# arclab-hku/ESVIO

Measured on AMD Instinct MI355X. Metric: Mevents/s through time-surface+detect+track @640x480, higher is better.
Workload: dtype f64 timestamps / u8 images / f32 LK sums in the reference build's order

## Files before the change

### esvio_amd/csrc/fe_kernels.hip

```cpp
#include "fe_kernels.h"
#include "fe_mc.h"

#include <algorithm>
#include <cstdio>
#include <cstdlib>
#include <cstring>
#include <tuple>
#include <type_traits>

namespace esvio {

namespace {
template <typename... P, typename... A>
void launch_k(void (*kernel)(P...), dim3 grid, dim3 block, unsigned shmem, hipStream_t s, A... args) {
  static_assert(sizeof...(P) == sizeof...(A), "argument count");
  hipLaunchKernelGGL(kernel, grid, block, shmem, s, args...);
}
}

__device__ __forceinline__ int lane_id() { return threadIdx.x & 63; }

__device__ __forceinline__ double ev_time(uint32_t sec, uint32_t nsec) {
  return __dadd_rn((double)sec, __dmul_rn(1e-9, (double)nsec));
}
// ... 1739 lines not shown
  float scale, corr;
};
__device__ __forceinline__ RedLane red_lane(int lane) {
  RedLane r;
  r.take_b = (lane & 2) != 0;
  const bool hi = (lane & 1) != 0;
  r.off = hi ? 12u : 0u;
  r.wid = hi ? 20u : 12u;
  r.scale = hi ? 0x1p-8f : 0x1p-20f;
  r.corr = hi ? -(float)(1 << 22) * 0x1p-8f : 0.f;
  return r;
}
template <int CTRL>
__device__ __forceinline__ float quad_bcast(float v) {
  return __int_as_float(__builtin_amdgcn_update_dpp(0, __float_as_int(v), CTRL, 0xf, 0xf, true));
}
constexpr int kRedSeed = 1 << 28;
__device__ __forceinline__ void wave_sum2_exact(int a, int b, const RedLane& rl, float& fa, float& fb) {
  a = xor_add_dpp(a, 0xB1);
  b = xor_add_dpp(b, 0xB1);
  a = xor_add_dpp(a, 0x4E);
  b = xor_add_dpp(b, 0x4E);
  a = xor_add_dpp(a, 0x141);
  b = xor_add_dpp(b, 0x141);
  const uint32_t v = (uint32_t)(rl.take_b ? b : a);
  int x = (int)__builtin_amdgcn_ubfe(v, rl.off, rl.wid);
  x = xor_add_dpp(x, 0x128);
  x = xor16_add(x);
  x = xor32_add(x);
  const float t = __fmaf_rn((float)x, rl.scale, rl.corr);
  const float u = t + quad_bcast<0xB1>(t);
  fa = quad_bcast<0x00>(u);
  fb = quad_bcast<0xAA>(u);
}

typedef short ss2 __attribute__((ext_vector_type(2)));
typedef unsigned short us2 __attribute__((ext_vector_type(2)));
__device__ __forceinline__ uint32_t pack16(int lo, int hi) {
  return __builtin_amdgcn_perm((uint32_t)hi, (uint32_t)lo, 0x05040100u);
}
__device__ __forceinline__ int sdot2(uint32_t a, uint32_t b, int c) {
  return __builtin_amdgcn_sdot2(__builtin_bit_cast(ss2, a), __builtin_bit_cast(ss2, b), c, false);
}

__device__ __forceinline__ bool wave_any(bool c) { return __builtin_amdgcn_ballot_w64(c) != 0; }
typedef unsigned long long lanemask_t;
__device__ __forceinline__ lanemask_t bal(bool c) { return __builtin_amdgcn_ballot_w64(c); }

struct LkCall {
  PyrDesc P;
  PyrDesc N;
  int max_level;
  int max_count;
  double eps2;
  int flags;
};

struct LkRegionLane {
  int ry[(kLkRegDw + 63) / 64], rb[(kLkRegDw + 63) / 64];
};
__device__ __forceinline__ LkRegionLane lk_region_lane(int lane) {
  LkRegionLane r;
#pragma unroll
  for (int k = 0; k < (kLkRegDw + 63) / 64; k++) {
    const int d = min(k * 64 + lane, kLkRegDw - 1);
    r.ry[k] = d / (kLkRegW / 4);
    r.rb[k] = 4 * (d - r.ry[k] * (kLkRegW / 4));
  }
  return r;
}
__device__ __forceinline__ void lk_region_load(const uint8_t* J, int stride, int rows, int wx, int wy,
                                               int lane, const LkRegionLane& rl, int& rx0, int& ry0,
                                               uint32_t (&reg)[(kLkRegDw + 63) / 64]) {
  rx0 = (wx - kLkMargin) & ~3;
  ry0 = wy - kLkMargin;
  const int sx = __builtin_amdgcn_readfirstlane(rx0), sy = __builtin_amdgcn_readfirstlane(ry0);
  if (sx >= -kPad && sx + kLkRegW <= stride - kPad && sy >= -kPad && sy + kLkRegH <= rows + kPad) {
    const uint8_t* base = J + (ptrdiff_t)sy * stride + sx;
#pragma unroll
    for (int k = 0; k < (kLkRegDw + 63) / 64; k++) {
      uint32_t off;
      asm("v_mad_u32_u24 %0, %1, %2, %3" : "=v"(off) : "v"(rl.ry[k]), "s"(stride), "v"(rl.rb[k]));
      reg[k] = *(const uint32_t*)(base + off);
    }
    return;
  }
#pragma unroll
  for (int k = 0; k < (kLkRegDw + 63) / 64; k++) {
    int gy = ry0 + rl.ry[k], gx = rx0 + rl.rb[k];
    gy = min(max(gy, -kPad), rows + kPad - 1);
    gx = min(max(gx, -kPad), stride - kPad - 4);
    reg[k] = *(const uint32_t*)(J + (ptrdiff_t)gy * stride + gx);
  }
}
__device__ __forceinline__ void lk_region_store(uint32_t* regJ, int lane,
                                                const uint32_t (&reg)[(kLkRegDw + 63) / 64]) {
  __builtin_amdgcn_fence(__ATOMIC_SEQ_CST, "wavefront");
#pragma unroll
  for (int k = 0; k < (kLkRegDw + 63) / 64; k++) {
    regJ[k * 64 + lane] = reg[k];
  }
  __builtin_amdgcn_fence(__ATOMIC_SEQ_CST, "wavefront");
}

__device__ __forceinline__ float lk_chain_walk(const float* T) {
  float acc = 0.f;
  float c[5], nx[5];
#pragma unroll
  for (int q = 0; q < 5; q++) c[q] = T[q];
#pragma unroll
  for (int y = 0; y < kLkWin; y++) {
    const int yn = y + 1 < kLkWin ? y + 1 : y;
#pragma unroll
    for (int q = 0; q < 5; q++) nx[q] = T[yn * 5 + q];
#pragma unroll
    for (int q = 0; q < 5; q++) acc = __fadd_rn(acc, c[q]);
#pragma unroll
    for (int q = 0; q < 5; q++) c[q] = nx[q];
  }
  return acc;
}

constexpr int kLkChainsA = 15;
constexpr int kLkChainWordsA = kLkWin * 5;
constexpr int kLkTypeWordsA = 5 * kLkChainWordsA;
constexpr int kLkTermLevelA = kLkChainsA * kLkChainWordsA;
constexpr int kLkTermWordsA = kMaxLevels * kLkTermLevelA;
static_assert(kMaxLevels * 16 <= 64, "one DPP row of walkers per level");

typedef __attribute__((address_space(3))) float lds_f32;
__device__ __forceinline__ int lk_term_word_A(int row, int x) {
  const int chain = x < 16 ? (x & 3) : x < kLkWin ? 4 : (x & 3);
  const int slot = x < 16 ? (x >> 2) : x < kLkWin ? x - 16 : 4;
  return (chain * kLkWin + row) * 5 + slot;
}
template <int NP>
__device__ __forceinline__ void lk_float_terms_A(const uint32_t (&ta)[NP], int L, const int* pIx, const int* pIy) {
#pragma unroll
  for (int k = 0; k < NP; k++) {
    lds_f32* d = (lds_f32*)(uintptr_t)ta[k] + L * kLkTermLevelA;
    const float fx = (float)pIx[k], fy = (float)pIy[k];
    d[0] = __fmul_rn(fx, fx);
    d[kLkTypeWordsA] = __fmul_rn(fx, fy);
    d[2 * kLkTypeWordsA] = __fmul_rn(fy, fy);
  }
}
__device__ __forceinline__ float lk_float_walk_A(const float* TA, int lane) {
  __builtin_amdgcn_fence(__ATOMIC_SEQ_CST, "wavefront", "local");
  const int c = (lane & 15) < kLkChainsA ? (lane & 15) : 0;
  return lk_chain_walk(TA + ((lane >> 4) * kLkChainsA + c) * kLkChainWordsA);
}
template <int CTRL>
__device__ __forceinline__ float dpp_row_f32(float v) {
  return __int_as_float(__builtin_amdgcn_update_dpp(0, __float_as_int(v), CTRL, 0xf, 0xf, true));
}
__device__ __forceinline__ float lk_float_sums_A(float acc, float& a11, float& a12, float& a22) {
  const float kScale = 1.f / (float)(1 << 20);
  const float s1 = __fadd_rn(acc, dpp_row_f32<0x102>(acc));
  const float s2 = __fadd_rn(s1, dpp_row_f32<0x101>(s1));
  const float s3 = __fadd_rn(dpp_row_f32<0x104>(acc), s2);
  const float out = __fmul_rn(s3, kScale);
  a11 = out;
  a12 = dpp_row_f32<0x105>(out);
  a22 = dpp_row_f32<0x10A>(out);
  return out;
}

constexpr int kF32SegStore = 12;
constexpr int kF32VecSegs = 4, kF32VecTerms = 11;
constexpr int kF32TailSegs = 12, kF32TailTerms = 9;
constexpr int kF32VecWords = kF32VecSegs * kF32SegStore;
constexpr int kF32CompStride = 4 * kF32VecWords;
constexpr int kF32TailBase = 8 * kF32VecWords;
constexpr int kF32ZeroSeg = kF32TailBase + kF32TailSegs * kF32SegStore;
constexpr int kF32Dump = kF32TailBase + kF32CompStride + kF32TailSegs * kF32SegStore;
constexpr int kF32TermWords = kF32Dump + kF32CompStride + 64;
static_assert(kF32ZeroSeg + kF32SegStore <= kF32TailBase + kF32CompStride, "zero segment inside tail b1's padding");
constexpr unsigned long long kF32Walkers = 0x0FFFFFFFFFFF0FFFull;

struct LkLaneF32 {
  uint32_t wb[5];
  uint32_t rb;
  uint32_t ta[8];
  bool run2;
};
__device__ __forceinline__ LkLaneF32 lk_lane_f32(int lane_in, uint32_t ta_base ) {
  const int lane = lane_in < 63 ? lane_in : 62;
  LkLaneF32 r;
  const int row = lane / 3;
  const int run = lane - row * 3;
  r.run2 = run == 2;
#pragma unroll
  for (int k = 0; k < 8; k++) r.ta[k] = ta_base + 4u * (uint32_t)lk_term_word_A(row, run * 8 + k);
#pragma unroll
  for (int j = 0; j < 5; j++) {
    int w = kF32Dump + lane;
    if (run < 2 && j < 4) {
      const int idx = 2 * row + run;
      w = j * kF32VecWords + (idx / kF32VecTerms) * kF32SegStore + idx % kF32VecTerms;
    } else if (run == 2) {
      const int idx = 5 * row + j;
      w = kF32TailBase + (idx / kF32TailTerms) * kF32SegStore + idx % kF32TailTerms;
    }
    r.wb[j] = (uint32_t)w * 4u;
  }
  const int wrow = lane_in >> 4, l16 = lane_in & 15;
  int rw = kF32ZeroSeg;
  if (wrow == 0 || wrow == 3) {
    if (l16 < kF32TailSegs) rw = kF32TailBase + (wrow == 3 ? kF32CompStride : 0) + l16 * kF32SegStore;
  } else {
    rw = ((wrow - 1) * 4 + (l16 & 3)) * kF32VecWords + (l16 >> 2) * kF32SegStore;
  }
  r.rb = (uint32_t)rw * 4u;
  return r;
}
template <int CTRL, int ROWS, int BANKS>
__device__ __forceinline__ int dpp_add_masked(int v) {
  return v + __builtin_amdgcn_update_dpp(0, v, CTRL, ROWS, BANKS, false);
}

typedef __attribute__((address_space(3))) int lds_int;
typedef int i32x4 __attribute__((ext_vector_type(4)));
typedef __attribute__((address_space(3))) i32x4 lds_int4;

__device__ __forceinline__ void lk_float_sums_b(const int (&vx)[5], const int (&vy)[5], uint32_t tb, const LkLaneF32& ln,
                                                float& b1, float& b2) {
  __builtin_amdgcn_fence(__ATOMIC_SEQ_CST, "wavefront", "local");
#pragma unroll
  for (int j = 0; j < 5; j++) {
    lds_int* d = (lds_int*)(uintptr_t)(tb + ln.wb[j]);
    d[0] = vx[j];
    d[kF32CompStride] = vy[j];
  }
  __builtin_amdgcn_fence(__ATOMIC_SEQ_CST, "wavefront", "local");
  int t[kF32SegStore];
  {
    const lds_int4* src = (const lds_int4*)(uintptr_t)(tb + ln.rb);
#pragma unroll
    for (int q = 0; q < kF32SegStore / 4; q++) {
      const i32x4 v = src[q];
      t[4 * q] = v.x;
      t[4 * q + 1] = v.y;
      t[4 * q + 2] = v.z;
      t[4 * q + 3] = v.w;
    }
  }
  int isum = 0;
  float f[kF32VecTerms];
#pragma unroll
  for (int i = 0; i < kF32VecTerms; i++) {
    isum += t[i];
    f[i] = (float)t[i];
  }
  int xa = isum, xb = isum;
  xa = dpp_add_masked<0x111, 0x9, 0xf>(xa);
  xb = dpp_add_masked<0x114, 0x6, 0xe>(xb);
  xa = dpp_add_masked<0x112, 0x9, 0xf>(xa);
  xb = dpp_add_masked<0x118, 0x6, 0xc>(xb);
  xa = dpp_add_masked<0x114, 0x9, 0xf>(xa);
  xa = dpp_add_masked<0x118, 0x9, 0xf>(xa);
  float guess = (float)(xa + xb - 2 * isum), end;
  for (;;) {
    float acc = guess;
#pragma unroll
    for (int i = 0; i < kF32VecTerms; i++) acc = __fadd_rn(acc, f[i]);
    end = acc;
    int s = __builtin_amdgcn_update_dpp(0, __float_as_int(acc), 0x111, 0x9, 0xf, false);
    s = __builtin_amdgcn_update_dpp(s, __float_as_int(acc), 0x114, 0x6, 0xe, false);
    const lanemask_t changed = bal((uint32_t)s != __float_as_uint(guess)) & kF32Walkers;
    guess = __int_as_float(s);
    if (!changed) break;
  }
  int e = __float_as_int(end);
  float q = __fadd_rn(end, __int_as_float(__builtin_amdgcn_update_dpp(0, e, 0x4E, 0xf, 0xf, false)));
  q = __fadd_rn(q, __int_as_float(__builtin_amdgcn_update_dpp(0, __float_as_int(q), 0xB1, 0xf, 0xf, false)));
  const int qi = __float_as_int(q);
  const float kScale = 1.f / (float)(1 << 20);
  const float t1 = __int_as_float(__builtin_amdgcn_readlane(e, 11)), t2 = __int_as_float(__builtin_amdgcn_readlane(e, 59));
  const float v1 = __int_as_float(__builtin_amdgcn_readlane(qi, 28)), v2 = __int_as_float(__builtin_amdgcn_readlane(qi, 44));
  b1 = __fmul_rn(__fadd_rn(t1, v1), kScale);
  b2 = __fmul_rn(__fadd_rn(t2, v2), kScale);
}

typedef float f2 __attribute__((ext_vector_type(2)));
typedef __attribute__((address_space(3))) const uint32_t lds_cu32;

__device__ __forceinline__ uint32_t mad_u24_regw(uint32_t oy, uint32_t ox) {
  uint32_t r;
  static_assert(kLkRegW <= 64, "inline constant");
  asm("v_mad_u32_u24 %0, %1, %2, %3" : "=v"(r) : "v"(oy), "n"(kLkRegW), "v"(ox));
  return r;
}
__device__ __forceinline__ int sdot2_zero(uint32_t a, uint32_t b) {
  int r;
  asm("v_dot2_i32_i16 %0, %1, %2, 0" : "=v"(r) : "v"(a), "v"(b));
  return r;
}
__device__ __forceinline__ int sdot2_seed(uint32_t a, uint32_t b, int seed) {
  int r;
  asm("v_dot2_i32_i16 %0, %1, %2, %3" : "=v"(r) : "v"(a), "v"(b), "s"(seed));
  return r;
}

template <int ACCUM>
__device__ __forceinline__ void lk_point(const LkCall& c, const float2 prev0, const float2 init,
                                         uint32_t* regJ, uint32_t term_base, float* acc_ta, const LkLaneF32* lnf, int lane,
                                         float2& np_out, int& st_out) {
  constexpr int WIN = kLkWin, NP = ACCUM == 2 ? 8 : 7, NPP = 4, NL = kMaxLevels;
  const float halfWin = (WIN - 1) * 0.5f;
  const int W_BITS = 14;
  const RedLane rl = red_lane(lane);
  const bool on = ACCUM == 2 || lane < 63;
  const int plane = ACCUM == 2 ? min(lane, 62) : lane;
  const int row = on ? plane / 3 : 0;
  const int x0 = on ? (plane - row * 3) * NP : 0;
  const int lane_bo = row * kLkRegW + x0;
  const LkRegionLane rgl = lk_region_lane(lane);

  uint32_t pIp[NL][NPP], pIxp[NL][NPP], pIyp[NL][NPP];
  uint32_t pIxB[NL], pIyB[NL];
  bool win_ok[NL], eig_ok[NL];
  float A11[NL], A12[NL], A22[NL], Dinv[NL];
  {
    constexpr int NW = (NP + 1 + 3) / 4;
    typedef uint32_t __attribute__((aligned(1))) u32_unaligned;
    uint32_t t0[NL][NW], t1[NL][NW];
    int g0[NL][NP + 1], g1[NL][NP + 1];
    uint32_t W0p[NL], W1p[NL];
    if (ACCUM == 2) __builtin_amdgcn_fence(__ATOMIC_SEQ_CST, "wavefront", "local");
#pragma unroll
    for (int L = 0; L < NL; L++) {
      win_ok[L] = false;
      eig_ok[L] = false;
      if (L > c.max_level) continue;
      const int cols = c.P.w[L], rows = c.P.h[L], stride = c.P.stride[L];
      const float sc = 1.f / (float)(1 << L);
      const float prevX = prev0.x * sc - halfWin, prevY = prev0.y * sc - halfWin;
      const float flx = floorf(prevX), fly = floorf(prevY);
      const int iprevX = (int)flx, iprevY = (int)fly;
      win_ok[L] = !(iprevX < -WIN || iprevX >= cols || iprevY < -WIN || iprevY >= rows);
      const float fa = prevX - flx, fb = prevY - fly;
      const int w00 = __float2int_rn((1.f - fa) * (1.f - fb) * (1 << W_BITS));
      const int w01 = __float2int_rn(fa * (1.f - fb) * (1 << W_BITS));
      const int w10 = __float2int_rn((1.f - fa) * fb * (1 << W_BITS));
      const int w11 = (1 << W_BITS) - w00 - w01 - w10;
      W0p[L] = pack16(w00, w10);
      W1p[L] = pack16(w01, w11);
      const int lx = min(max(iprevX, -WIN), cols - 1), ly = min(max(iprevY, -WIN), rows - 1);
      const ptrdiff_t o = (ptrdiff_t)(kPad + row + ly) * stride + kPad + lx + x0;
      const uint8_t* s0 = c.P.img[L] + o;
      const uint8_t* s1 = s0 + stride;
      const int* d0 = (const int*)c.P.deriv[L] + o;
      const int* d1 = d0 + stride;
#pragma unroll
      for (int q = 0; q < NW; q++) {
        t0[L][q] = ((const u32_unaligned*)s0)[q];
        t1[L][q] = ((const u32_unaligned*)s1)[q];
      }
#pragma unroll
      for (int k = 0; k <= NP; k++) {
        g0[L][k] = d0[k];
        g1[L][k] = d1[k];
      }
    }
#pragma unroll
    for (int L = 0; L < NL; L++) {
      if (L > c.max_level) continue;
      int sA11 = kRedSeed, sA12 = kRedSeed, sA22 = kRedSeed;
      int pI[2 * NPP], pIx[2 * NPP], pIy[2 * NPP];
#pragma unroll
      for (int k = NP; k < 2 * NPP; k++) pI[k] = pIx[k] = pIy[k] = 0;
      uint32_t vI[NP + 1], vX[NP + 1], vY[NP + 1];
#pragma unroll
      for (int k = 0; k <= NP; k++) {
        const uint32_t sel = 0x0c000c00u | ((uint32_t)(4 + (k & 3)) << 16) | (uint32_t)(k & 3);
        vI[k] = __builtin_amdgcn_perm(t1[L][k >> 2], t0[L][k >> 2], sel);
        vX[k] = __builtin_amdgcn_perm((uint32_t)g1[L][k], (uint32_t)g0[L][k], 0x05040100u);
        vY[k] = __builtin_amdgcn_perm((uint32_t)g1[L][k], (uint32_t)g0[L][k], 0x07060302u);
      }
#pragma unroll
      for (int k = 0; k < NP; k++) {
        const int ival = sdot2(vI[k + 1], W1p[L], sdot2_seed(vI[k], W0p[L], 1 << (W_BITS - 5 - 1))) >> (W_BITS - 5);
        const int ixval = sdot2(vX[k + 1], W1p[L], sdot2_seed(vX[k], W0p[L], 1 << (W_BITS - 1))) >> W_BITS;
        const int iyval = sdot2(vY[k + 1], W1p[L], sdot2_seed(vY[k], W0p[L], 1 << (W_BITS - 1))) >> W_BITS;
        const bool col_ok = ACCUM == 2 ? (k < WIN - 16 || !lnf->run2) : on;
        pI[k] = ival;
        pIx[k] = col_ok ? ixval : 0;
        pIy[k] = col_ok ? iyval : 0;
        if (ACCUM != 2) {
          sA11 += __mul24(pIx[k], pIx[k]);
          sA12 += __mul24(pIx[k], pIy[k]);
          sA22 += __mul24(pIy[k], pIy[k]);
        }
      }
#pragma unroll
      for (int m = 0; m < NPP; m++) {
        const int a = ACCUM == 2 ? m : 2 * m, b = ACCUM == 2 ? m + 4 : 2 * m + 1;
        pIp[L][m] = pack16(pI[a], pI[b]);
        pIxp[L][m] = pack16(pIx[a], pIx[b]);
        pIyp[L][m] = pack16(pIy[a], pIy[b]);
      }
      if (ACCUM == 2) {
        if (lnf->run2) {
          pIxp[L][0] = pack16(pIx[0], 0);
          pIyp[L][0] = pack16(pIy[0], 0);
        }
        pIxB[L] = pack16(0, pIx[4]);
        pIyB[L] = pack16(0, pIy[4]);
      }
      if (ACCUM == 2) {
        lk_float_terms_A<8>(lnf->ta, L, pIx, pIy);
      } else {
        float fdummy;
        wave_sum2_exact(sA11, sA12, rl, A11[L], A12[L]);
        wave_sum2_exact(sA22, kRedSeed, rl, A22[L], fdummy);
      }
    }
    if (ACCUM == 2) {
      float a11, a12, a22;
      const float out = lk_float_sums_A(lk_float_walk_A(acc_ta, lane), a11, a12, a22);
      const float D = a11 * a22 - a12 * a12;
      const float minEig = (a22 + a11 - sqrtf((a11 - a22) * (a11 - a22) + 4.f * a12 * a12)) / (float)(2 * WIN * WIN);
      const lanemask_t ok = bal(!(minEig < 1e-4f || D < 1.1920929e-07f ));
      const float dinv = 1.f / D;
#pragma unroll
      for (int L = 0; L < NL; L++) {
        if (L > c.max_level) continue;
        A11[L] = __int_as_float(__builtin_amdgcn_readlane(__float_as_int(out), 16 * L));
        A12[L] = __int_as_float(__builtin_amdgcn_readlane(__float_as_int(out), 16 * L + 5));
        A22[L] = __int_as_float(__builtin_amdgcn_readlane(__float_as_int(out), 16 * L + 10));
        Dinv[L] = __int_as_float(__builtin_amdgcn_readlane(__float_as_int(dinv), 16 * L));
        eig_ok[L] = (ok >> (16 * L)) & 1;
      }
    } else {
#pragma unroll
      for (int L = 0; L < NL; L++) {
        if (L > c.max_level) continue;
        const float D = A11[L] * A22[L] - A12[L] * A12[L];
        const float minEig =
            (A22[L] + A11[L] - sqrtf((A11[L] - A22[L]) * (A11[L] - A22[L]) + 4.f * A12[L] * A12[L])) /
            (float)(2 * WIN * WIN);
        eig_ok[L] = !(minEig < 1e-4f || D < 1.1920929e-07f );
        Dinv[L] = 1.f / D;
      }
    }
  }

  const float eps_lo = (float)(c.eps2 * (1.0 - 0x1p-20)), eps_hi = (float)(c.eps2 * (1.0 + 0x1p-20));
  const uint32_t regJ_b = (uint32_t)(uintptr_t)(__attribute__((address_space(3))) uint32_t*)regJ;
  float2 np = (c.flags & 4) ? init : make_float2(0.f, 0.f);
  int st = 1;
#pragma unroll
  for (int L = NL - 1; L >= 0; L--) {
    if (L > c.max_level) continue;
    const int cols = c.P.w[L], rows = c.P.h[L];
    const int stride = c.P.stride[L];
    const uint8_t* J = c.N.img[L] + (size_t)kPad * stride + kPad;
    const float sc = 1.f / (float)(1 << L);
    float nextX, nextY;
    if (L == c.max_level) {
      if (c.flags & 4) {
        nextX = np.x * sc;
        nextY = np.y * sc;
      } else {
        nextX = prev0.x * sc;
        nextY = prev0.y * sc;
      }
    } else {
      nextX = np.x * 2.f;
      nextY = np.y * 2.f;
    }
    np = make_float2(nextX, nextY);
    if (wave_any(!win_ok[L] || !eig_ok[L])) {
      if (L == 0) st = 0;
      continue;
    }
    f2 nxt = {nextX - halfWin, nextY - halfWin};
    f2 fl = {floorf(nxt.x), floorf(nxt.y)};
    int inx = (int)fl.x, iny = (int)fl.y;
    f2 d = {0.f, 0.f}, prevD = {__builtin_inff(), __builtin_inff()};
    int j = 0;
    bool level_done = c.max_count <= 0;
    if (wave_any(inx < -WIN || inx >= cols || iny < -WIN || iny >= rows)) {
      if (L == 0) st = 0;
      level_done = true;
    }
    while (!level_done) {
      int rx0, ry0;
      {
        uint32_t reg[(kLkRegDw + 63) / 64];
        lk_region_load(J, stride, rows, inx, iny, lane, rgl, rx0, ry0, reg);
        lk_region_store(regJ, lane, reg);
      }
      const int lox = max(rx0, -WIN), loy = max(ry0, -WIN);
      const uint32_t rngx = (uint32_t)(min(rx0 + (kLkRegW - (WIN + 1)), cols - 1) - lox);
      const uint32_t rngy = (uint32_t)(min(ry0 + (kLkRegH - (WIN + 1)), rows - 1) - loy);
      const uint32_t cbo = regJ_b + (uint32_t)lane_bo + mad_u24_regw((uint32_t)(loy - ry0), (uint32_t)(lox - rx0));
      uint32_t ox = (uint32_t)(inx - lox), oy = (uint32_t)(iny - loy);
      float d2 = 0.f;
      f2 osum = {0.f, 0.f};
      bool restage = false;
      for (;;) {
        for (;;) {
          const f2 fr = nxt - fl, ofr = 1.f - fr;
          const float kMagic = 8388608.f, kW = (float)(1 << W_BITS);
          const f2 cross = fr * f2{ofr.y, ofr.x};
          const f2 bc = __builtin_elementwise_fma(cross, f2{kW, kW}, f2{kMagic, kMagic});
          const uint32_t b00 = __float_as_uint(__fmaf_rn(ofr.x * ofr.y, kW, kMagic));
          const uint32_t b01 = __float_as_uint(bc.x);
          const uint32_t b10 = __float_as_uint(bc.y);
          const uint32_t iw11 = ((1u << W_BITS) + 3u * 0x4B000000u) - (b00 + b01 + b10);
          const uint32_t W0 = __builtin_amdgcn_perm(b10, b00, 0x05040100u);
          const uint32_t W1 = __builtin_amdgcn_perm(iw11, b01, 0x05040100u);
          const uint32_t bo = mad_u24_regw(oy, ox) + cbo;
          lds_cu32* rp = (lds_cu32*)(uintptr_t)(bo & ~3u);
          const uint32_t a0 = rp[0], a1 = rp[1], a2 = rp[2];
          const uint32_t c0 = rp[kLkRegW / 4], c1 = rp[kLkRegW / 4 + 1], c2 = rp[kLkRegW / 4 + 2];
          uint32_t w0[3], w1[3];
          w0[0] = __builtin_amdgcn_alignbyte(a1, a0, bo);
          w0[1] = __builtin_amdgcn_alignbyte(a2, a1, bo);
          w1[0] = __builtin_amdgcn_alignbyte(c1, c0, bo);
          w1[1] = __builtin_amdgcn_alignbyte(c2, c1, bo);
          if (NP == 8) {
            w0[2] = __builtin_amdgcn_alignbyte(a2, a2, bo);
            w1[2] = __builtin_amdgcn_alignbyte(c2, c2, bo);
          }
          uint32_t t[2 * NPP], vc[NP + 1];
#pragma unroll
          for (int k = 0; k <= NP; k++) {
            const uint32_t sel = 0x0c000c00u | ((uint32_t)(4 + (k & 3)) << 16) | (uint32_t)(k & 3);
            vc[k] = __builtin_amdgcn_perm(w1[k >> 2], w0[k >> 2], sel);
          }
#pragma unroll
          for (int k = 0; k < NP; k++)
            t[k] = (uint32_t)sdot2(vc[k + 1], W1, sdot2_seed(vc[k], W0, 1 << (W_BITS - 5 - 1)));
#pragma unroll
          for (int k = NP; k < 2 * NPP; k++) t[k] = 0;
          float b1, b2;
          if (ACCUM == 2) {
            int vx[5], vy[5];
#pragma unroll
            for (int m = 0; m < NPP; m++) {
              const uint32_t hi8 = __builtin_amdgcn_perm(t[m + 4], t[m], 0x06050201u);
              const us2 val = __builtin_bit_cast(us2, hi8) >> (unsigned short)1;
              const uint32_t diff = __builtin_bit_cast(uint32_t, __builtin_bit_cast(ss2, val) - __builtin_bit_cast(ss2, pIp[L][m]));
              vx[m] = sdot2_zero(diff, pIxp[L][m]);
              vy[m] = sdot2_zero(diff, pIyp[L][m]);
              if (m == 0) {
                vx[4] = sdot2_zero(diff, pIxB[L]);
                vy[4] = sdot2_zero(diff, pIyB[L]);
              }
            }
            lk_float_sums_b(vx, vy, term_base, *lnf, b1, b2);
          } else {
            int sb1 = 0, sb2 = 0;
#pragma unroll
            for (int m = 0; m < NPP; m++) {
              const uint32_t hi8 = __builtin_amdgcn_perm(t[2 * m + 1], t[2 * m], 0x06050201u);
              const us2 val = __builtin_bit_cast(us2, hi8) >> (unsigned short)1;
              const uint32_t diff = __builtin_bit_cast(uint32_t, __builtin_bit_cast(ss2, val) - __builtin_bit_cast(ss2, pIp[L][m]));
              if (m == 0) {
                sb1 = sdot2_seed(diff, pIxp[L][m], kRedSeed);
                sb2 = sdot2_seed(diff, pIyp[L][m], kRedSeed);
              } else {
                sb1 = sdot2(diff, pIxp[L][m], sb1);
                sb2 = sdot2(diff, pIyp[L][m], sb2);
              }
            }
            wave_sum2_exact(sb1, sb2, rl, b1, b2);
          }
          d = f2{(A12[L] * b2 - A22[L] * b1) * Dinv[L], (A12[L] * b1 - A11[L] * b2) * Dinv[L]};
          d2 = __fmaf_rn(d.x, d.x, d.y * d.y);
          osum = d + prevD;
          prevD = d;
          nxt += d;
          fl = f2{floorf(nxt.x), floorf(nxt.y)};
          inx = (int)fl.x;
          iny = (int)fl.y;
          ox = (uint32_t)(inx - lox);
          oy = (uint32_t)(iny - loy);
          j++;
          const float thr = j >= c.max_count ? __builtin_inff() : eps_hi;
          if (bal(!(d2 >= thr)) | bal(fmaxf(fabsf(osum.x), fabsf(osum.y)) <= 0.01f) | bal(ox > rngx) | bal(oy > rngy)) break;
        }
        asm volatile("" : "+v"(d2), "+v"(ox), "+v"(oy));
        asm volatile("" : "+v"(osum));
        np = make_float2(nxt.x + halfWin, nxt.y + halfWin);
        lanemask_t conv = bal(d2 <= eps_lo);
        if (__builtin_expect((bal(d2 > eps_lo) & bal(d2 < eps_hi)) != 0, 0)) {
          asm volatile("; fp64 tie-break" ::: "memory");
          conv = bal((double)d.x * (double)d.x + (double)d.y * (double)d.y <= c.eps2);
        }
        if (conv) {
          level_done = true;
          break;
        }
        if (bal(fabsf(osum.x) <= 0.01f) & bal(fabsf(osum.y) <= 0.01f)) {
          np.x -= d.x * 0.5f;
          np.y -= d.y * 0.5f;
          level_done = true;
          break;
        }
        if (j >= c.max_count) {
          level_done = true;
          break;
        }
        if (wave_any(inx < -WIN || inx >= cols || iny < -WIN || iny >= rows)) {
          if (L == 0) st = 0;
          level_done = true;
          break;
        }
        if (wave_any(ox > rngx || oy > rngy)) {
          restage = true;
          break;
        }
      }
      (void)restage;
    }
    if (st && L == 0) {
      const float fx = np.x - halfWin, fy = np.y - halfWin;
      const int ix = (int)floorf(fx), iy = (int)floorf(fy);
      if (ix < -WIN || ix >= cols || iy < -WIN || iy >= rows) st = 0;
    }
  }
  np_out = np;
  st_out = st;
}

struct LkKernelArgs {
  LkCall fwd;
  LkCall back;
  int have_back;
  const float2* prev_pts;
  const float2* init_pts;
  float2* next_pts;
  uint8_t* status;
  float2* back_pts;
  uint8_t* back_status;
  const int* n_ptr;
  int n_max;
  const unsigned long long* poll_slots;
  const unsigned long long* poll_done;
  uint32_t poll_seq;
  int poll_from;
  int* poll_err;
  unsigned long long* chain_out;
  const unsigned long long* chain_in;
  uint32_t chain_seq;
  unsigned long long poll_ticks, chain_ticks;
  const uint32_t* gate_ptr;
  uint32_t gate_val;
};

__device__ __forceinline__ void chain_publish(const LkKernelArgs& a, int pt, int lane, float2 p, int alive) {
  if (!a.chain_out || lane != 0) return;
  const unsigned long long hi = (unsigned long long)((a.chain_seq << 2) | (uint32_t)(alive ? 1 : 0)) << 32;
  __hip_atomic_store(&a.chain_out[2 * pt], hi | __float_as_uint(p.x), __ATOMIC_RELAXED, __HIP_MEMORY_SCOPE_AGENT);
  __hip_atomic_store(&a.chain_out[2 * pt + 1], hi | __float_as_uint(p.y), __ATOMIC_RELAXED,
                     __HIP_MEMORY_SCOPE_AGENT);
}

template <int ACCUM>
__device__ __forceinline__ void lk_kernel_body(const LkKernelArgs& a, uint32_t (*regJ_s)[kLkRegStore], uint32_t acc_t,
                                               float* acc_ta, const LkLaneF32* lnf) {
  const int wave = threadIdx.x >> 6, lane = lane_id();
  const int pt = blockIdx.x * kLkWaves + wave;
  const int n = a.n_ptr ? *a.n_ptr : a.n_max;
  if (pt >= a.n_max) return;
  if (pt >= n) {
    chain_publish(a, pt, lane, make_float2(0.f, 0.f), 0);
    return;
  }
  float2 prev0;
  if (a.chain_in) {
    const unsigned long long t0 = wall_clock64();
    unsigned long long vx, vy;
    if (!a.chain_ticks) {
      if (lane == 0) *a.poll_err = 1;
      return;
    }
    for (;;) {
      vx = __hip_atomic_load(&a.chain_in[2 * pt], __ATOMIC_RELAXED, __HIP_MEMORY_SCOPE_AGENT);
      vy = __hip_atomic_load(&a.chain_in[2 * pt + 1], __ATOMIC_RELAXED, __HIP_MEMORY_SCOPE_AGENT);
      if ((uint32_t)(vx >> 34) == a.chain_seq && (uint32_t)(vy >> 34) == a.chain_seq) break;
      if (wall_clock64() - t0 > a.chain_ticks) {
        if (lane == 0) *a.poll_err = 1;
        return;
      }
      __builtin_amdgcn_s_sleep(8);
    }
    if (!((uint32_t)(vx >> 32) & 1u)) {
      if (lane == 0) {
        a.status[pt] = 0;
        if (a.have_back) a.back_status[pt] = 0;
      }
      return;
    }
    prev0 = make_float2(__uint_as_float((uint32_t)vx), __uint_as_float((uint32_t)vy));
    if (a.gate_ptr) {
      for (;;) {
        const uint32_t gv = __hip_atomic_load(a.gate_ptr, __ATOMIC_RELAXED, __HIP_MEMORY_SCOPE_AGENT);
        if ((int)(gv - a.gate_val) >= 0) break;
        if (wall_clock64() - t0 > a.chain_ticks) {
          if (lane == 0) *a.poll_err = 1;
          return;
        }
        __builtin_amdgcn_s_sleep(8);
      }
      __builtin_amdgcn_fence(__ATOMIC_ACQUIRE, "agent");
    }
  } else if (a.poll_slots && pt >= a.poll_from) {
    const unsigned long long t0 = wall_clock64();
    unsigned long long v;
    for (;;) {
      v = __hip_atomic_load(&a.poll_slots[pt], __ATOMIC_RELAXED, __HIP_MEMORY_SCOPE_AGENT);
      if ((uint32_t)(v >> 32) == a.poll_seq) break;
      const unsigned long long d = __hip_atomic_load(a.poll_done, __ATOMIC_RELAXED, __HIP_MEMORY_SCOPE_AGENT);
      if ((uint32_t)(d >> 32) == a.poll_seq && pt >= (int)(uint32_t)d) {
        chain_publish(a, pt, lane, make_float2(0.f, 0.f), 0);
        return;
      }
      if (wall_clock64() - t0 > a.poll_ticks) {
        if (lane == 0) *a.poll_err = 1;
        chain_publish(a, pt, lane, make_float2(0.f, 0.f), 0);
        return;
      }
      __builtin_amdgcn_s_sleep(16);
    }
    prev0 = make_float2((float)(uint32_t)(v & 0xffffu), (float)(uint32_t)((v >> 16) & 0xffffu));
  } else {
    prev0 = a.prev_pts[pt];
  }
  const float2 init = (a.fwd.flags & 4) ? a.init_pts[pt] : make_float2(0.f, 0.f);
  float2 np;
  int st;
  lk_point<ACCUM>(a.fwd, prev0, init, regJ_s[wave], acc_t, acc_ta, lnf, lane, np, st);
  chain_publish(a, pt, lane, np, st);
  if (lane == 0) {
    a.next_pts[pt] = np;
    a.status[pt] = (uint8_t)st;
  }
  if (a.have_back) {
    float2 bp;
    int bs;
    lk_point<ACCUM>(a.back, np, prev0, regJ_s[wave], acc_t, acc_ta, lnf, lane, bp, bs);
    if (lane == 0) {
      a.back_pts[pt] = bp;
      a.back_status[pt] = (uint8_t)bs;
    }
  }
}

__global__ __launch_bounds__(64 * kLkWaves) void k_lk(LkKernelArgs a) {
  __shared__ __attribute__((aligned(16))) uint32_t regJ_s[kLkWaves][kLkRegStore];
  lk_kernel_body<1>(a, regJ_s, 0u, nullptr, nullptr);
}
__global__ __launch_bounds__(64 * kLkWaves) void k_lk_f32(LkKernelArgs a) {
  __shared__ __attribute__((aligned(16))) uint32_t regJ_s[kLkWaves][kLkRegStore];
  __shared__ __attribute__((aligned(16))) int term_all[kLkWaves][kF32TermWords];
  __shared__ __attribute__((aligned(16))) float term_a[kLkWaves][kLkTermWordsA];
  const int wave = threadIdx.x >> 6, lane = threadIdx.x & 63;
  for (int i = lane; i < kF32TermWords; i += 64) term_all[wave][i] = 0;
  {
    const int l = lane < 63 ? lane : 62, t = l / kLkWin, rw = l - t * kLkWin;
    float* z = term_a[wave] + 5 * t * kLkChainWordsA + rw * 5 + 4;
#pragma unroll
    for (int L = 0; L < kMaxLevels; L++)
#pragma unroll
      for (int k = 0; k < 4; k++) z[L * kLkTermLevelA + k * kLkChainWordsA] = 0.f;
  }
  __builtin_amdgcn_fence(__ATOMIC_SEQ_CST, "wavefront", "local");
  const LkLaneF32 lnf =
      lk_lane_f32(lane, (uint32_t)(uintptr_t)(__attribute__((address_space(3))) float*)term_a[wave]);
  const uint32_t tb = (uint32_t)(uintptr_t)(__attribute__((address_space(3))) int*)term_all[wave];
  lk_kernel_body<2>(a, regJ_s, tb, term_a[wave], &lnf);
}

void launch_lk(hipStream_t s, const LkArgs& f, const LkArgs* b, float2* back_pts,
               uint8_t* back_status) {
  if (f.n_max <= 0) return;
  LkKernelArgs a;
  a.fwd.P = f.P;
  a.fwd.N = f.N;
  a.fwd.max_level = f.max_level;
  a.fwd.max_count = f.max_count;
  a.fwd.eps2 = f.eps2;
  a.fwd.flags = f.flags;
  a.have_back = b ? 1 : 0;
  a.back = a.fwd;
  if (b) {
    a.back.P = b->P;
    a.back.N = b->N;
    a.back.max_level = b->max_level;
    a.back.max_count = b->max_count;
    a.back.eps2 = b->eps2;
    a.back.flags = b->flags;
  }
  a.prev_pts = f.prev_pts;
  a.init_pts = f.init_pts;
  a.next_pts = f.next_pts;
  a.status = f.status;
  a.back_pts = back_pts;
  a.back_status = back_status;
  a.n_ptr = f.n_ptr;
  a.n_max = f.n_max;
  a.poll_slots = f.poll_slots;
  a.poll_done = f.poll_done;
  a.poll_seq = f.poll_seq;
  a.poll_from = f.poll_from;
  a.poll_err = f.poll_err;
  a.chain_out = f.chain_out;
  a.chain_in = f.chain_in;
  a.chain_seq = f.chain_seq;
  a.poll_ticks = f.poll_ticks;
  a.chain_ticks = f.chain_ticks;
  a.gate_ptr = f.gate_ptr;
  a.gate_val = f.gate_val;
  if (f.accum == 2)
    launch_k(k_lk_f32, dim3((a.n_max + kLkWaves - 1) / kLkWaves), dim3(64 * kLkWaves), 0, s, a);
  else
    launch_k(k_lk, dim3((a.n_max + kLkWaves - 1) / kLkWaves), dim3(64 * kLkWaves), 0, s, a);
}

__constant__ int8_t c_small[16][2] = {{0, 3},  {1, 3},   {2, 2},   {3, 1},  {3, 0},  {3, -1},
                                      {2, -2}, {1, -3},  {0, -3},  {-1, -3}, {-2, -2}, {-3, -1},
                                      {-3, 0}, {-3, 1},  {-2, 2},  {-1, 3}};
__constant__ int8_t c_large[20][2] = {{0, 4},   {1, 4},   {2, 3},   {3, 2},  {4, 1},  {4, 0},  {4, -1},
                                      {3, -2},  {2, -3},  {1, -4},  {0, -4}, {-1, -4}, {-2, -3}, {-3, -2},
                                      {-4, -1}, {-4, 0},  {-4, 1},  {-3, 2}, {-2, 3},  {-1, 4}};

template <int N>
struct RingRanks {
  unsigned long long lo, hi;
  __device__ __forceinline__ int get(int i) const {
    if (N <= 16) return (int)((lo >> (4 * i)) & 15ull);
    return i < 10 ? (int)((lo >> (5 * i)) & 31ull) : (int)((hi >> (5 * (i - 10))) & 31ull);
  }
};

template <int N, int KMIN, int KMAX>
__device__ __forceinline__ bool arc_ring_ranks(const double (&v)[N]) {
  int r[N];
#pragma unroll
  for (int i = 0; i < N; i++) r[i] = 0;
#pragma unroll
  for (int i = 1; i < N; i++)
#pragma unroll
    for (int j = 0; j < i; j++) {
      r[i] += v[j] < v[i] ? 1 : 0;
      r[j] += v[i] < v[j] ? 1 : 0;
    }
  RingRanks<N> rk;
  rk.lo = 0;
  rk.hi = 0;
#pragma unroll
  for (int i = 0; i < N; i++) {
    if (N <= 16) rk.lo |= (unsigned long long)r[i] << (4 * i);
    else if (i < 10) rk.lo |= (unsigned long long)r[i] << (5 * i);
    else rk.hi |= (unsigned long long)r[i] << (5 * (i - 10));
  }
  int segment_new_min_t = r[0];
  int arc_right_idx = 0;
#pragma unroll
  for (int i = 1; i < N; i++)
    if (r[i] > segment_new_min_t) {
      segment_new_min_t = r[i];
      arc_right_idx = i;
    }
  int arc_left_idx = arc_right_idx == 0 ? N - 1 : arc_right_idx - 1;
  arc_right_idx = arc_right_idx == N - 1 ? 0 : arc_right_idx + 1;
  int arc_left_value = rk.get(arc_left_idx);
  int arc_right_value = rk.get(arc_right_idx);
  int arc_left_min_t = arc_left_value;
  int arc_right_min_t = arc_right_value;
  int newest_segment_size = KMIN;
#pragma unroll
  for (int iteration = 1; iteration < N; iteration++) {
    const bool right = arc_right_value > arc_left_value;
    const int val = right ? arc_right_value : arc_left_value;
    const int mn = right ? arc_right_min_t : arc_left_min_t;
    if (iteration < KMIN) {
      if (mn < segment_new_min_t) segment_new_min_t = mn;
    } else if (val >= segment_new_min_t) {
      newest_segment_size = iteration + 1;
      if (mn < segment_new_min_t) segment_new_min_t = mn;
    }
    if (right) {
      arc_right_idx = arc_right_idx == N - 1 ? 0 : arc_right_idx + 1;
      arc_right_value = rk.get(arc_right_idx);
      if (arc_right_value < arc_right_min_t) arc_right_min_t = arc_right_value;
    } else {
      arc_left_idx = arc_left_idx == 0 ? N - 1 : arc_left_idx - 1;
      arc_left_value = rk.get(arc_left_idx);
      if (arc_left_value < arc_left_min_t) arc_left_min_t = arc_left_value;
    }
  }
  return (newest_segment_size <= KMAX) ||
         ((newest_segment_size >= (N - KMAX)) && (newest_segment_size <= (N - KMIN)));
}

constexpr int kArcRegion = 256;

__device__ __forceinline__ uint32_t block_list_slot(bool take, uint32_t* wave_cnt, uint32_t* total,
                                                    unsigned long long counted = 0, uint32_t* wave_cnt2 = nullptr,
                                                    uint32_t* total2 = nullptr) {
  const int wave = threadIdx.x >> 6, lane = lane_id();
  const unsigned long long m = __ballot(take);
  if (lane == 0) {
    wave_cnt[wave] = __popcll(m);
    if (wave_cnt2) wave_cnt2[wave] = __popcll(counted);
  }
  __syncthreads();
  uint32_t base = 0, tot = 0, tot2 = 0;
#pragma unroll
  for (int w = 0; w < kArcBlock / 64; w++) {
    if (w < wave) base += wave_cnt[w];
    tot += wave_cnt[w];
    if (wave_cnt2) tot2 += wave_cnt2[w];
  }
  *total = tot;
  if (total2) *total2 = tot2;
  return base + __popcll(m & ((1ull << lane) - 1ull));
}

__global__ __launch_bounds__(256) void k_arc_mark(const uint4* __restrict__ ev, uint32_t n, int W, int H,
                                                  uint8_t* __restrict__ touched) {
  for (uint32_t i = blockIdx.x * blockDim.x + threadIdx.x; i < n; i += gridDim.x * blockDim.x) {
    const uint32_t xy = ((const uint32_t*)ev)[4 * (size_t)i], pw = ((const uint32_t*)ev)[4 * (size_t)i + 3];
    const uint32_t x = xy & 0xffffu, y = xy >> 16;
    if (x < (uint32_t)W && y < (uint32_t)H) touched[2u * (y * (uint32_t)W + x) + ((pw & 0xffu) ? 1u : 0u)] = 1;
  }
}

__global__ __launch_bounds__(kArcBlock) void k_arc_map(ArcArgs a) {
  __shared__ uint16_t list_b[2 * kArcRegion];
  __shared__ uint32_t n_b;
  const uint32_t P = (uint32_t)a.W * (uint32_t)a.H;
  const uint32_t pair0 = blockIdx.x * (2u * kArcRegion);
  if (threadIdx.x == 0) n_b = 0;
  __syncthreads();
  {
    const uint32_t px = (pair0 >> 1) + threadIdx.x;
    uint32_t f = 0;
    if (px < P) {
      f = ((const uint16_t*)a.touched)[px];
      if (f) ((uint16_t*)a.touched)[px] = 0;
    }
    if (threadIdx.x < (2 * kArcRegion) / 32) {
      const uint32_t w = (pair0 >> 5) + threadIdx.x;
      if (w < (2u * P + 31u) / 32u) a.cmap[w] = 0;
    }
    if (f) {
      const int y = (int)(px / (uint32_t)a.W), x = (int)(px - (uint32_t)y * (uint32_t)a.W);
      bool ok = !(x < a.border || x >= a.W - a.border || y < a.border || y >= a.H - a.border);
      ok = ok && x >= 4 && y >= 4 && x < a.W - 4 && y < a.H - 4;
      if (ok && a.ts) ok = (double)a.ts[(size_t)(y + kPad) * a.ts_stride + x + kPad] != a.ts_lk_threshold;
      if (ok) {
        const double2 Lv = a.L2[px];
        if ((f & 0x00ffu) && !(Lv.y > Lv.x)) list_b[atomicAdd(&n_b, 1u)] = (uint16_t)(2u * threadIdx.x);
        if ((f & 0xff00u) && !(Lv.x > Lv.y)) list_b[atomicAdd(&n_b, 1u)] = (uint16_t)(2u * threadIdx.x + 1u);
      }
    }
  }
  __syncthreads();
  const uint32_t nb = n_b;
  for (uint32_t i = threadIdx.x; i < nb; i += kArcBlock) {
    const uint32_t pair = pair0 + list_b[i], px = pair >> 1, pol = pair & 1u;
    const int y = (int)(px / (uint32_t)a.W), x = (int)(px - (uint32_t)y * (uint32_t)a.W);
    const double* S = (const double*)a.S2 + pol;
    double v16[16];
#pragma unroll
    for (int k = 0; k < 16; k++) v16[k] = S[2 * ((size_t)(y + c_small[k][1]) * a.W + (x + c_small[k][0]))];
    if (!arc_ring_ranks<16, 4, 6>(v16)) continue;
    double v20[20];
#pragma unroll
    for (int k = 0; k < 20; k++) v20[k] = S[2 * ((size_t)(y + c_large[k][1]) * a.W + (x + c_large[k][0]))];
    if (arc_ring_ranks<20, 5, 8>(v20)) atomicOr(&a.cmap[pair >> 5], 1u << (pair & 31));
  }
}

__global__ __launch_bounds__(kArcBlock) void k_arc_ev(ArcArgs a) {
  __shared__ uint32_t wave_cnt[kArcBlock / 64];
  const uint32_t i = blockIdx.x * kArcBlock + threadIdx.x;
  bool corner = false;
  uint32_t x = 0, y = 0;
  if (i < a.n) {
    const uint4 e = ((const uint4*)a.ev)[i];
    x = e.x & 0xffffu;
    y = e.x >> 16;
    if (x < (uint32_t)a.W && y < (uint32_t)a.H) {
      const int pol = (e.w & 0xffu) ? 1 : 0;
      const uint32_t px = y * (uint32_t)a.W + x;
      const uint32_t pair = 2u * px + (uint32_t)pol;
      bool ok = (a.cmap[pair >> 5] >> (pair & 31)) & 1u;
      if (ok && a.mask_bits) ok = !((a.mask_bits[y * a.wpr + (x >> 5)] >> (x & 31)) & 1u);
      if (ok) {
        const double t_last = ((const double*)a.L2)[2 * (size_t)px + pol];
        if (ev_time(e.y, e.z) > __dadd_rn(t_last, a.filter_threshold)) ok = false;
      }
      corner = ok;
    }
    if (a.flags) a.flags[i] = corner ? 1 : 0;
  }
  if (a.cand_cnt) {
    uint32_t total;
    const size_t pos = (size_t)blockIdx.x * kArcBlock + block_list_slot(corner, wave_cnt, &total);
    if (corner) {
      a.cand_xy[pos] = x | (y << 16);
      a.cand_idx[pos] = i;
      if (a.first_map) atomicMin(&a.first_map[y * (uint32_t)a.W + x], a.first_key | i);
    }
    if (threadIdx.x == 0) a.cand_cnt[blockIdx.x] = total;
  }
}

__global__ __launch_bounds__(256) void k_stage_pull(const uint4* __restrict__ src, uint4* __restrict__ dst, size_t n) {
  const size_t stride = (size_t)gridDim.x * blockDim.x;
  for (size_t i = (size_t)blockIdx.x * blockDim.x + threadIdx.x; i < n; i += stride) dst[i] = src[i];
}
constexpr int kStageDescLds = 1024;
__global__ __launch_bounds__(256) void k_stage_pull_packed(const uint8_t* __restrict__ src, uint4* __restrict__ dst, size_t n,
                                                           const uint2* __restrict__ desc, uint32_t epc) {
  __shared__ uint2 sd[kStageDescLds];
  const size_t nch = (n + epc - 1) / epc;
  const bool cached = nch <= (size_t)kStageDescLds;
  if (cached) {
    for (size_t k = threadIdx.x; k < nch; k += blockDim.x) sd[k] = desc[k];
    __syncthreads();
  }
  const size_t stride = (size_t)gridDim.x * blockDim.x;
  for (size_t i = (size_t)blockIdx.x * blockDim.x + threadIdx.x; i < n; i += stride) {
    const size_t c = i / epc, j = i - c * epc;
    const uint2 d = cached ? sd[c] : desc[c];
    const uint8_t* base = src + c * (size_t)epc * 16;
    if (d.y) {
      const uint2 v = ((const uint2*)base)[j];
      dst[i] = make_uint4(v.x, d.x + (v.y >> 31), v.y & 0x3fffffffu, (v.y >> 30) & 1u);
    } else {
      dst[i] = ((const uint4*)base)[j];
    }
  }
}
void launch_stage_pull_packed(hipStream_t s, const void* pinned_src, void* dst, size_t bytes, const void* desc, uint32_t epc) {
  const size_t n = bytes / 16;
  if (!n) return;
  const unsigned grid = (unsigned)std::min<size_t>(64, (n + 255) / 256);
  launch_k(k_stage_pull_packed, dim3(grid), dim3(256), 0, s, (const uint8_t*)pinned_src, (uint4*)dst, n, (const uint2*)desc, epc);
}
void launch_stage_pull(hipStream_t s, const void* pinned_src, void* dst, size_t bytes) {
  const size_t n = bytes / 16;
  if (!n) return;
// ... 1131 lines not shown
```

Measured before the change: 2880.

## Roll LK pyramid level loop and forward/back passes to cut code size and registers

The coarse-to-fine pyramid level loop in lk_point is no longer unrolled. Per-level values are now chosen at runtime with select chains, or read with readlane from the kept vector values. The forward and backward LK calls are merged into one rolled loop that reads the call parameters directly from the kernarg segment, in the constant address space. Global pointer casts let the compiler emit global rather than flat loads. The aim is to shrink instruction footprint and register pressure, and so raise occupancy and reduce i-cache misses. The cost is extra select and readlane work per level and the loss of constant-folded level indices.

```diff
diff --git a/esvio_amd/csrc/fe_kernels.hip b/esvio_amd/csrc/fe_kernels.hip
--- a/esvio_amd/csrc/fe_kernels.hip
+++ b/esvio_amd/csrc/fe_kernels.hip
@@ -2065,8 +2065,26 @@
   return r;
 }
 
+typedef const __attribute__((address_space(4))) LkCall lk_call_k;
+template <typename T>
+__device__ __forceinline__ const T* lk_global(const T* p) {
+  return (const T*)(const __attribute__((address_space(1))) T*)p;
+}
+
+static_assert(kMaxLevels == 4, "lk_level_pick");
+template <typename T>
+__device__ __forceinline__ T lk_level_pick(T v0, T v1, T v2, T v3, int L) {
+  T r = v0;
+  r = L == 1 ? v1 : r;
+  r = L == 2 ? v2 : r;
+  r = L == 3 ? v3 : r;
+  return r;
+}
+#define LK_LEVEL_PICK(v, L) lk_level_pick((v)[0], (v)[1], (v)[2], (v)[3], (L))
+#define LK_LEVEL_PICK2(v, m, L) lk_level_pick((v)[0][m], (v)[1][m], (v)[2][m], (v)[3][m], (L))
+
 template <int ACCUM>
-__device__ __forceinline__ void lk_point(const LkCall& c, const float2 prev0, const float2 init,
+__device__ __forceinline__ void lk_point(lk_call_k& c, const float2 prev0, const float2 init,
                                          uint32_t* regJ, uint32_t term_base, float* acc_ta, const LkLaneF32* lnf, int lane,
                                          float2& np_out, int& st_out) {
   constexpr int WIN = kLkWin, NP = ACCUM == 2 ? 8 : 7, NPP = 4, NL = kMaxLevels;
@@ -2084,6 +2102,7 @@
   uint32_t pIxB[NL], pIyB[NL];
   bool win_ok[NL], eig_ok[NL];
   float A11[NL], A12[NL], A22[NL], Dinv[NL];
+  float outA = 0.f, dinvA = 0.f;
   {
     constexpr int NW = (NP + 1 + 3) / 4;
     typedef uint32_t __attribute__((aligned(1))) u32_unaligned;
@@ -2111,9 +2130,9 @@
       W1p[L] = pack16(w01, w11);
       const int lx = min(max(iprevX, -WIN), cols - 1), ly = min(max(iprevY, -WIN), rows - 1);
       const ptrdiff_t o = (ptrdiff_t)(kPad + row + ly) * stride + kPad + lx + x0;
-      const uint8_t* s0 = c.P.img[L] + o;
+      const uint8_t* s0 = lk_global(c.P.img[L]) + o;
       const uint8_t* s1 = s0 + stride;
-      const int* d0 = (const int*)c.P.deriv[L] + o;
+      const int* d0 = (const int*)lk_global(c.P.deriv[L]) + o;
       const int* d1 = d0 + stride;
 #pragma unroll
       for (int q = 0; q < NW; q++) {
@@ -2185,14 +2204,11 @@
       const float D = a11 * a22 - a12 * a12;
       const float minEig = (a22 + a11 - sqrtf((a11 - a22) * (a11 - a22) + 4.f * a12 * a12)) / (float)(2 * WIN * WIN);
       const lanemask_t ok = bal(!(minEig < 1e-4f || D < 1.1920929e-07f ));
-      const float dinv = 1.f / D;
+      outA = out;
+      dinvA = 1.f / D;
 #pragma unroll
       for (int L = 0; L < NL; L++) {
         if (L > c.max_level) continue;
-        A11[L] = __int_as_float(__builtin_amdgcn_readlane(__float_as_int(out), 16 * L));
-        A12[L] = __int_as_float(__builtin_amdgcn_readlane(__float_as_int(out), 16 * L + 5));
-        A22[L] = __int_as_float(__builtin_amdgcn_readlane(__float_as_int(out), 16 * L + 10));
-        Dinv[L] = __int_as_float(__builtin_amdgcn_readlane(__float_as_int(dinv), 16 * L));
         eig_ok[L] = (ok >> (16 * L)) & 1;
       }
     } else {
@@ -2213,13 +2229,19 @@
   const uint32_t regJ_b = (uint32_t)(uintptr_t)(__attribute__((address_space(3))) uint32_t*)regJ;
   float2 np = (c.flags & 4) ? init : make_float2(0.f, 0.f);
   int st = 1;
-#pragma unroll
+  uint32_t level_ok = 0;
+#pragma unroll
+  for (int L = 0; L < NL; L++) {
+    if (L > c.max_level) continue;
+    if (!wave_any(!win_ok[L] || !eig_ok[L])) level_ok |= 1u << L;
+  }
+#pragma unroll 1
   for (int L = NL - 1; L >= 0; L--) {
     if (L > c.max_level) continue;
     const int cols = c.P.w[L], rows = c.P.h[L];
     const int stride = c.P.stride[L];
-    const uint8_t* J = c.N.img[L] + (size_t)kPad * stride + kPad;
-    const float sc = 1.f / (float)(1 << L);
+    const uint8_t* J = lk_global(c.N.img[L]) + (size_t)kPad * stride + kPad;
+    const float sc = __int_as_float((127 - L) << 23);
     float nextX, nextY;
     if (L == c.max_level) {
       if (c.flags & 4) {
@@ -2234,9 +2256,30 @@
       nextY = np.y * 2.f;
     }
     np = make_float2(nextX, nextY);
-    if (wave_any(!win_ok[L] || !eig_ok[L])) {
+    if (!((level_ok >> L) & 1u)) {
       if (L == 0) st = 0;
       continue;
+    }
+    uint32_t cIp[NPP], cIxp[NPP], cIyp[NPP], cIxB = 0, cIyB = 0;
+#pragma unroll
+    for (int m = 0; m < NPP; m++) {
+      cIp[m] = LK_LEVEL_PICK2(pIp, m, L);
+      cIxp[m] = LK_LEVEL_PICK2(pIxp, m, L);
+      cIyp[m] = LK_LEVEL_PICK2(pIyp, m, L);
+    }
+    float cA11, cA12, cA22, cDinv;
+    if (ACCUM == 2) {
+      cIxB = LK_LEVEL_PICK(pIxB, L);
+      cIyB = LK_LEVEL_PICK(pIyB, L);
+      cA11 = __int_as_float(__builtin_amdgcn_readlane(__float_as_int(outA), 16 * L));
+      cA12 = __int_as_float(__builtin_amdgcn_readlane(__float_as_int(outA), 16 * L + 5));
+      cA22 = __int_as_float(__builtin_amdgcn_readlane(__float_as_int(outA), 16 * L + 10));
+      cDinv = __int_as_float(__builtin_amdgcn_readlane(__float_as_int(dinvA), 16 * L));
+    } else {
+      cA11 = LK_LEVEL_PICK(A11, L);
+      cA12 = LK_LEVEL_PICK(A12, L);
+      cA22 = LK_LEVEL_PICK(A22, L);
+      cDinv = LK_LEVEL_PICK(Dinv, L);
     }
     f2 nxt = {nextX - halfWin, nextY - halfWin};
     f2 fl = {floorf(nxt.x), floorf(nxt.y)};
@@ -2306,12 +2349,12 @@
             for (int m = 0; m < NPP; m++) {
               const uint32_t hi8 = __builtin_amdgcn_perm(t[m + 4], t[m], 0x06050201u);
               const us2 val = __builtin_bit_cast(us2, hi8) >> (unsigned short)1;
-              const uint32_t diff = __builtin_bit_cast(uint32_t, __builtin_bit_cast(ss2, val) - __builtin_bit_cast(ss2, pIp[L][m]));
-              vx[m] = sdot2_zero(diff, pIxp[L][m]);
-              vy[m] = sdot2_zero(diff, pIyp[L][m]);
+              const uint32_t diff = __builtin_bit_cast(uint32_t, __builtin_bit_cast(ss2, val) - __builtin_bit_cast(ss2, cIp[m]));
+              vx[m] = sdot2_zero(diff, cIxp[m]);
+              vy[m] = sdot2_zero(diff, cIyp[m]);
               if (m == 0) {
-                vx[4] = sdot2_zero(diff, pIxB[L]);
-                vy[4] = sdot2_zero(diff, pIyB[L]);
+                vx[4] = sdot2_zero(diff, cIxB);
+                vy[4] = sdot2_zero(diff, cIyB);
               }
             }
             lk_float_sums_b(vx, vy, term_base, *lnf, b1, b2);
@@ -2321,18 +2364,18 @@
             for (int m = 0; m < NPP; m++) {
               const uint32_t hi8 = __builtin_amdgcn_perm(t[2 * m + 1], t[2 * m], 0x06050201u);
               const us2 val = __builtin_bit_cast(us2, hi8) >> (unsigned short)1;
-              const uint32_t diff = __builtin_bit_cast(uint32_t, __builtin_bit_cast(ss2, val) - __builtin_bit_cast(ss2, pIp[L][m]));
+              const uint32_t diff = __builtin_bit_cast(uint32_t, __builtin_bit_cast(ss2, val) - __builtin_bit_cast(ss2, cIp[m]));
               if (m == 0) {
-                sb1 = sdot2_seed(diff, pIxp[L][m], kRedSeed);
-                sb2 = sdot2_seed(diff, pIyp[L][m], kRedSeed);
+                sb1 = sdot2_seed(diff, cIxp[m], kRedSeed);
+                sb2 = sdot2_seed(diff, cIyp[m], kRedSeed);
               } else {
-                sb1 = sdot2(diff, pIxp[L][m], sb1);
-                sb2 = sdot2(diff, pIyp[L][m], sb2);
+                sb1 = sdot2(diff, cIxp[m], sb1);
+                sb2 = sdot2(diff, cIyp[m], sb2);
               }
             }
             wave_sum2_exact(sb1, sb2, rl, b1, b2);
           }
-          d = f2{(A12[L] * b2 - A22[L] * b1) * Dinv[L], (A12[L] * b1 - A11[L] * b2) * Dinv[L]};
+          d = f2{(cA12 * b2 - cA22 * b1) * cDinv, (cA12 * b1 - cA11 * b2) * cDinv};
           d2 = __fmaf_rn(d.x, d.x, d.y * d.y);
           osum = d + prevD;
           prevD = d;
@@ -2494,22 +2537,27 @@
   } else {
     prev0 = a.prev_pts[pt];
   }
-  const float2 init = (a.fwd.flags & 4) ? a.init_pts[pt] : make_float2(0.f, 0.f);
-  float2 np;
-  int st;
-  lk_point<ACCUM>(a.fwd, prev0, init, regJ_s[wave], acc_t, acc_ta, lnf, lane, np, st);
-  chain_publish(a, pt, lane, np, st);
-  if (lane == 0) {
-    a.next_pts[pt] = np;
-    a.status[pt] = (uint8_t)st;
-  }
-  if (a.have_back) {
-    float2 bp;
-    int bs;
-    lk_point<ACCUM>(a.back, np, prev0, regJ_s[wave], acc_t, acc_ta, lnf, lane, bp, bs);
-    if (lane == 0) {
-      a.back_pts[pt] = bp;
-      a.back_status[pt] = (uint8_t)bs;
+  float2 from = prev0;
+  float2 start = (a.fwd.flags & 4) ? a.init_pts[pt] : make_float2(0.f, 0.f);
+  const int passes = a.have_back ? 2 : 1;
+#pragma unroll 1
+  for (int pass = 0; pass < passes; pass++) {
+    const auto* ka = (const __attribute__((address_space(4))) LkKernelArgs*)__builtin_amdgcn_kernarg_segment_ptr();
+    lk_call_k& c = pass ? ka->back : ka->fwd;
+    float2 np;
+    int st;
+    lk_point<ACCUM>(c, from, start, regJ_s[wave], acc_t, acc_ta, lnf, lane, np, st);
+    if (pass == 0) {
+      chain_publish(a, pt, lane, np, st);
+      if (lane == 0) {
+        a.next_pts[pt] = np;
+        a.status[pt] = (uint8_t)st;
+      }
+      start = from;
+      from = np;
+    } else if (lane == 0) {
+      a.back_pts[pt] = np;
+      a.back_status[pt] = (uint8_t)st;
     }
   }
 }
```

After: 2750. 0.955x the previous value.
